# Oscar-W-Chen/gpu-ai-inference-server

Measured on AMD Instinct MI355X. Metric: images/sec, DenseNet-121 fp32, batch 32 per GPU, device-resident inputs, higher is better.
Workload: dtype f32; 1 GPU; DenseNet-121 fp32 batch=32 per GPU, synthetic 3x224x224 inputs (BASELINE configs[1]); synthetic ONNX graph + seeded random weights (reference model file is not in the mount); global_batch=32, per_gpu_batch=32, parallelism=dp1 (independent batch shards)

## Files before the change

gpu-ai-inference-server_amd/csrc/kernels_wino.hip:

```cpp
#include <hip/hip_runtime.h>

#include <algorithm>
#include <cstdlib>
#include <type_traits>

#include "device_util.h"
#include "kernels.h"
#include "launch_util.h"

namespace ie {

__global__ void winograd_weights_kernel(const float* __restrict__ w, float* __restrict__ u, const int Cout, const int Cin) {
    const int idx = blockIdx.x * blockDim.x + threadIdx.x;
    if (idx >= Cout * Cin) return;
    const int co = idx / Cin, ci = idx - co * Cin;
    float g[3][3];
#pragma unroll
    for (int a = 0; a < 3; ++a)
#pragma unroll
        for (int b = 0; b < 3; ++b) g[a][b] = w[((co * 3 + a) * 3 + b) * Cin + ci];
    float t[4][3];
#pragma unroll
    for (int b = 0; b < 3; ++b) {
        t[0][b] = g[0][b];
        t[1][b] = 0.5f * (g[0][b] + g[1][b] + g[2][b]);
        t[2][b] = 0.5f * (g[0][b] - g[1][b] + g[2][b]);
        t[3][b] = g[2][b];
    }
    const int ch8 = ci >> 3, hh = (ci >> 2) & 1, e = ci & 3;
#pragma unroll
    for (int i = 0; i < 4; ++i) {
        const float uu[4] = {t[i][0], 0.5f * (t[i][0] + t[i][1] + t[i][2]), 0.5f * (t[i][0] - t[i][1] + t[i][2]), t[i][2]};
#pragma unroll
        for (int j = 0; j < 4; ++j) {
            const int xi = 4 * i + j;
            u[((int64_t(xi) * (Cin >> 3) + ch8) * 64 + (hh * 32 + co)) * 4 + e] = uu[j];
        }
    }
}

__global__ void winograd_weights_x6_kernel(const float* __restrict__ w, unsigned short* __restrict__ dst, const int Cout, const int Cin) {
    const int idx = blockIdx.x * blockDim.x + threadIdx.x;
    if (idx >= Cout * Cin) return;
    const int co = idx / Cin, ci = idx - co * Cin;
    float g[3][3];
#pragma unroll
    for (int a = 0; a < 3; ++a)
#pragma unroll
        for (int b = 0; b < 3; ++b) g[a][b] = w[((co * 3 + a) * 3 + b) * Cin + ci];
    float t[4][3];
#pragma unroll
    for (int b = 0; b < 3; ++b) {
        t[0][b] = g[0][b];
        t[1][b] = 0.5f * (g[0][b] + g[1][b] + g[2][b]);
        t[2][b] = 0.5f * (g[0][b] - g[1][b] + g[2][b]);
        t[3][b] = g[2][b];
    }
    const int KB = Cin >> 4, kb = ci >> 4, lane = co + 32 * ((ci >> 3) & 1), e = ci & 7;
    const int64_t plane = int64_t(16) * 32 * Cin;
#pragma unroll
    for (int i = 0; i < 4; ++i) {
        const float uu[4] = {t[i][0], 0.5f * (t[i][0] + t[i][1] + t[i][2]), 0.5f * (t[i][0] - t[i][1] + t[i][2]), t[i][2]};
#pragma unroll
        for (int j = 0; j < 4; ++j) {
            const float x = uu[j];
            const unsigned h0 = __builtin_bit_cast(unsigned, x) & 0xffff0000u;
            const float r1 = x - __builtin_bit_cast(float, h0);
            const unsigned h1 = __builtin_bit_cast(unsigned, r1) & 0xffff0000u;
            const unsigned h2 = __builtin_bit_cast(unsigned, r1 - __builtin_bit_cast(float, h1));
            const int64_t off = ((int64_t(4 * i + j) * KB + kb) * 64 + lane) * 8 + e;
            dst[off] = static_cast<unsigned short>(h0 >> 16);
            dst[plane + off] = static_cast<unsigned short>(h1 >> 16);
            dst[2 * plane + off] = static_cast<unsigned short>(h2 >> 16);
        }
    }
}

hipError_t LaunchWinogradWeightsX6(const float* w, void* dst, int Cout, int Cin, hipStream_t stream) {
    if (Cout != 32 || (Cin % 16) || Cin <= 0) return hipErrorInvalidValue;
    const int total = Cout * Cin;
    winograd_weights_x6_kernel<<<dim3((total + 255) / 256), dim3(256), 0, stream>>>(w, static_cast<unsigned short*>(dst), Cout, Cin);
    return hipGetLastError();
}

hipError_t LaunchWinogradWeights(const float* w, float* u, int Cout, int Cin, hipStream_t stream) {
    if (Cout != 32 || (Cin % 16) || Cin <= 0) return hipErrorInvalidValue;
    const int total = Cout * Cin;
    winograd_weights_kernel<<<dim3((total + 255) / 256), dim3(256), 0, stream>>>(w, u, Cout, Cin);
    return hipGetLastError();
}

struct WinoGeom {
    int TR, TC;
    int TH, TW;
    int bry, brx;
};

template <int WAVES, bool X6 = false>
__global__ __launch_bounds__(64 * WAVES) __attribute__((amdgpu_waves_per_eu(2, (WAVES == 8 && !X6) ? 4 : 2))) void conv3x3_wino_kernel(const ConvArgs a, const WinoGeom g) {
    constexpr int NT = 64 * WAVES, CS = 16, LP = CS + 4, MP = 32 + 4, PITW = 1024 / NT;
    constexpr int NJ = 16 / WAVES;
    constexpr unsigned OOB = 0x80000000u;
    extern __shared__ __attribute__((aligned(16))) float smem_wino[];
    const int WR = 2 * g.TR + 2, WC = 2 * g.TC + 2, npx = WR * WC;
    const int win_floats = (npx * LP + 3) & ~3;
    float* const sWin = smem_wino;
    float* const sM = smem_wino;

    const int tid = threadIdx.x, lane = tid & 63, r = lane & 31, hh = lane >> 5;
    const int wave = __builtin_amdgcn_readfirstlane(tid >> 6);
    const int Cin = a.in.c, H = a.in.h, W = a.in.w;
    const int ipitch = int(a.in.sw), opitch = int(a.out.sw);
    int bid = blockIdx.x;
    const int bx = bid % g.brx; bid /= g.brx;
    const int by = bid % g.bry;
    const int b = bid / g.bry;
    const int ty0 = by * g.TR, tx0 = bx * g.TC;
    const int ntr = min(g.TR, g.TH - ty0), ntc = min(g.TC, g.TW - tx0);
    const int y0 = 2 * ty0 - 1, x0 = 2 * tx0 - 1;
    const int ntiles = g.TR * g.TC;

    const __amdgpu_buffer_rsrc_t rs_in = __builtin_amdgcn_make_buffer_rsrc(a.in.p, 0, int(a.in_bytes), kBufferRsrcFlags);
    const __amdgpu_buffer_rsrc_t rs_u = __builtin_amdgcn_make_buffer_rsrc(const_cast<float*>(a.wfrag), 0, 16 * 32 * Cin * 4, kBufferRsrcFlags);

    const int items = npx * 4;
    int woff[PITW];
#pragma unroll
    for (int i = 0; i < PITW; ++i) {
        const int it = tid + i * NT;
        int off = -1;
        if (it < items) {
            const int px = it >> 2, q = it & 3;
            const int wy = px / WC, wx = px - wy * WC;
            const int y = y0 + wy, x = x0 + wx;
            if (unsigned(y) < unsigned(H) && unsigned(x) < unsigned(W)) off = ((b * H + y) * W + x) * ipitch + q * 4;
        }
        woff[i] = off;
    }
    unsigned wvo[PITW];
    float* wlds[2][PITW];
#pragma unroll
    for (int i = 0; i < PITW; ++i) {
        const int it = tid + i * NT;
        wvo[i] = woff[i] >= 0 ? unsigned(woff[i]) * 4u : OOB;
#pragma unroll
        for (int bf = 0; bf < 2; ++bf) wlds[bf][i] = sWin + bf * win_floats + (it >> 2) * LP + (it & 3) * 4;
    }
    f32x4 pvA[PITW], pvB[PITW];
    const int nslices = Cin / CS, nstages = 2 * nslices;
    auto issue_window = [&](f32x4 (&pv)[PITW], int s) {
#pragma unroll
        for (int i = 0; i < PITW; ++i)
            pv[i] = __builtin_bit_cast(f32x4, __builtin_amdgcn_raw_buffer_load_b128(rs_in, wvo[i], (s < nslices ? s : nslices - 1) * CS * 4, 0));
    };
    auto commit_window = [&](const f32x4 (&pv)[PITW], int buf) {
#pragma unroll
        for (int i = 0; i < PITW; ++i)
            if (tid + i * NT < items) *reinterpret_cast<f32x4*>(wlds[buf][i]) = pv[i];
    };
    const int wi = wave / (WAVES / 4), jh = wave % (WAVES / 4);
    const int ra = wi == 0 ? 0 : wi == 2 ? 2 : 1, rb = wi == 2 ? 1 : wi == 3 ? 3 : 2;
    const float sg = wi == 1 ? 1.f : -1.f;
    constexpr int NC = NJ == 4 ? 4 : 3;
    const int ltr = r / g.TC, ltc = r - ltr * g.TC;
    const int col0 = NJ == 4 ? 0 : jh;
    const int dA = ((2 * ltr + ra) * WC + 2 * ltc + col0) * LP + hh * 4, dB = ((2 * ltr + rb) * WC + 2 * ltc + col0) * LP + hh * 4;
    f32x16 acc[NJ];
#pragma unroll
    for (int xl = 0; xl < NJ; ++xl)
#pragma unroll
        for (int e = 0; e < 16; ++e) acc[xl][e] = 0.f;
    if constexpr (X6) {
        static_assert(NJ == 2, "the split variant is written for eight waves");
        const __amdgpu_buffer_rsrc_t rs_ux = __builtin_amdgcn_make_buffer_rsrc(const_cast<void*>(a.w16), 0, 3 * 16 * 32 * Cin * 2, kBufferRsrcFlags);
        const int KB = Cin >> 4;
        const int plane_b = 16 * 32 * Cin * 2;
        u32x4 ux0[NJ][3], ux1[NJ][3];
        auto issue_ux = [&](u32x4 (&ux)[NJ][3], int sl) {
            const int kb = sl < nslices ? sl : nslices - 1;
#pragma unroll
            for (int xl = 0; xl < NJ; ++xl)
#pragma unroll
                for (int p = 0; p < 3; ++p) ux[xl][p] = __builtin_amdgcn_raw_buffer_load_b128(rs_ux, unsigned(lane) * 16u, p * plane_b + ((NJ * wave + xl) * KB + kb) * 1024, 0);
        };
        const float* const qdA[2] = {sWin + dA + hh * 4, sWin + win_floats + dA + hh * 4};
        const float* const qdB[2] = {sWin + dB + hh * 4, sWin + win_floats + dB + hh * 4};
        f32x4 xra[3][2], xrb[3][2];
        auto read_dx = [&](int buf) {
#pragma unroll
            for (int c = 0; c < 3; ++c)
#pragma unroll
                for (int q = 0; q < 2; ++q) {
                    xra[c][q] = *reinterpret_cast<const f32x4*>(qdA[buf] + c * LP + q * 4);
                    xrb[c][q] = *reinterpret_cast<const f32x4*>(qdB[buf] + c * LP + q * 4);
                }
        };
        const float ka0 = jh == 0 ? 1.f : -1.f, ka1 = jh == 0 ? 0.f : 1.f, ka2 = jh == 0 ? -1.f : 0.f;
        const float kb0 = jh == 0 ? 0.f : 1.f, kb1 = jh == 0 ? 1.f : 0.f, kb2 = jh == 0 ? 1.f : -1.f;
        u32x4 axA[NJ][3], axB[NJ][3];
        auto make_ax = [&](u32x4 (&ax)[NJ][3]) {
            f32x4 v[NJ][2];
#pragma unroll
            for (int q = 0; q < 2; ++q) {
                f32x4 m[3];
#pragma unroll
                for (int c = 0; c < 3; ++c) m[c] = xra[c][q] + sg * xrb[c][q];
                v[0][q] = ka0 * m[0] + ka1 * m[1] + ka2 * m[2];
                v[1][q] = kb0 * m[0] + kb1 * m[1] + kb2 * m[2];
            }
#pragma unroll
            for (int xl = 0; xl < NJ; ++xl) {
                unsigned h0[8], h1[8], h2[8];
#pragma unroll
                for (int e = 0; e < 8; ++e) {
                    const float x = v[xl][e >> 2][e & 3];
                    h0[e] = __builtin_bit_cast(unsigned, x);
                    const float r1 = x - __builtin_bit_cast(float, h0[e] & 0xffff0000u);
                    h1[e] = __builtin_bit_cast(unsigned, r1);
                    h2[e] = __builtin_bit_cast(unsigned, r1 - __builtin_bit_cast(float, h1[e] & 0xffff0000u));
                }
#pragma unroll
                for (int d = 0; d < 4; ++d) {
                    ax[xl][0][d] = __builtin_amdgcn_perm(h0[2 * d + 1], h0[2 * d], 0x07060302u);
                    ax[xl][1][d] = __builtin_amdgcn_perm(h1[2 * d + 1], h1[2 * d], 0x07060302u);
                    ax[xl][2][d] = __builtin_amdgcn_perm(h2[2 * d + 1], h2[2 * d], 0x07060302u);
                }
            }
        };
        auto mfmas_x = [&](const u32x4 (&ax)[NJ][3], const u32x4 (&ux)[NJ][3]) {
#pragma unroll
            for (int xl = 0; xl < NJ; ++xl) {
                const bf16x8 a0 = __builtin_bit_cast(bf16x8, ax[xl][0]), a1 = __builtin_bit_cast(bf16x8, ax[xl][1]), a2 = __builtin_bit_cast(bf16x8, ax[xl][2]);
                const bf16x8 b0 = __builtin_bit_cast(bf16x8, ux[xl][0]), b1 = __builtin_bit_cast(bf16x8, ux[xl][1]), b2 = __builtin_bit_cast(bf16x8, ux[xl][2]);
                acc[xl] = __builtin_amdgcn_mfma_f32_32x32x16_bf16(a2, b0, acc[xl], 0, 0, 0);
                acc[xl] = __builtin_amdgcn_mfma_f32_32x32x16_bf16(a1, b1, acc[xl], 0, 0, 0);
                acc[xl] = __builtin_amdgcn_mfma_f32_32x32x16_bf16(a0, b2, acc[xl], 0, 0, 0);
                acc[xl] = __builtin_amdgcn_mfma_f32_32x32x16_bf16(a1, b0, acc[xl], 0, 0, 0);
                acc[xl] = __builtin_amdgcn_mfma_f32_32x32x16_bf16(a0, b1, acc[xl], 0, 0, 0);
                acc[xl] = __builtin_amdgcn_mfma_f32_32x32x16_bf16(a0, b0, acc[xl], 0, 0, 0);
            }
        };
        issue_window(pvA, 0);
        issue_window(pvB, 1);
        issue_ux(ux0, 0);
        commit_window(pvA, 0);
        issue_window(pvA, 2);
        __syncthreads();
        read_dx(0);
        make_ax(axA);
        commit_window(pvB, 1);
        issue_window(pvB, 3);
        __syncthreads();
        auto xslice = [&](auto parity, int sl, u32x4 (&a_cur)[NJ][3], u32x4 (&a_nxt)[NJ][3], u32x4 (&u_cur)[NJ][3], u32x4 (&u_nxt)[NJ][3], f32x4 (&pv_c)[PITW]) {
            constexpr int P = decltype(parity)::value;
            read_dx(P ^ 1);
            issue_ux(u_nxt, sl + 1);
            mfmas_x(a_cur, u_cur);
            make_ax(a_nxt);
#pragma unroll
            for (int i = 0; i < 6 * NJ; ++i) {
                __builtin_amdgcn_sched_group_barrier(0x008, 1, 0);
                __builtin_amdgcn_sched_group_barrier(0x002, 14, 0);
            }
            commit_window(pv_c, P);
            issue_window(pv_c, sl + 4);
            __syncthreads();
        };
        for (int sl = 0; sl < nslices; sl += 2) {
            xslice(std::integral_constant<int, 0>{}, sl, axA, axB, ux0, ux1, pvA);
            xslice(std::integral_constant<int, 1>{}, sl + 1, axB, axA, ux1, ux0, pvB);
        }
    } else {
    const int c8n = Cin >> 3;
    u32x4 ub0[NJ], ub1[NJ];
    auto issue_u = [&](u32x4 (&ub)[NJ], int h) {
#pragma unroll
        for (int xl = 0; xl < NJ; ++xl)
            ub[xl] = __builtin_amdgcn_raw_buffer_load_b128(rs_u, unsigned(lane) * 16u, ((NJ * wave + xl) * c8n + (h < nstages ? h : nstages - 1)) * 1024, 0);
    };
    f32x4 dra[NC], drb[NC];
    const float* const pdA[2] = {sWin + dA, sWin + win_floats + dA};
    const float* const pdB[2] = {sWin + dB, sWin + win_floats + dB};
    auto read_d = [&](int buf, int half) {
#pragma unroll
        for (int c = 0; c < NC; ++c) {
            dra[c] = *reinterpret_cast<const f32x4*>(pdA[buf] + half * 8 + c * LP);
            drb[c] = *reinterpret_cast<const f32x4*>(pdB[buf] + half * 8 + c * LP);
        }
    };
    f32x4 af[NJ];
    auto make_af = [&]() {
        f32x4 m[NC];
#pragma unroll
        for (int c = 0; c < NC; ++c) m[c] = dra[c] + sg * drb[c];
        if constexpr (NJ == 4) {
            af[0] = m[0] - m[2];
            af[1] = m[1] + m[2];
            af[2] = m[2] - m[1];
            af[3] = m[1] - m[3];
        } else if (jh == 0) {
            af[0] = m[0] - m[2];
            af[1] = m[1] + m[2];
        } else {
            af[0] = m[1] - m[0];
            af[1] = m[0] - m[2];
        }
    };
    auto mfmas = [&](const u32x4 (&ub)[NJ]) {
        f32x4 ac[NJ];
#pragma unroll
        for (int xl = 0; xl < NJ; ++xl) ac[xl] = af[xl];
#pragma unroll
        for (int e = 0; e < 4; ++e)
#pragma unroll
            for (int xl = 0; xl < NJ; ++xl)
                acc[xl] = __builtin_amdgcn_mfma_f32_32x32x2f32(ac[xl][e], __builtin_bit_cast(f32x4, ub[xl])[e], acc[xl], 0, 0, 0);
    };

    issue_window(pvA, 0);
    issue_window(pvB, 1);
    issue_u(ub0, 0);
    issue_u(ub1, 1);
    commit_window(pvA, 0);
    issue_window(pvA, 2);
    __syncthreads();
    read_d(0, 0);
    make_af();
    auto slice = [&](auto parity, int s, f32x4 (&pv_next)[PITW]) {
        constexpr int P = decltype(parity)::value;
        read_d(P, 1);
        commit_window(pv_next, P ^ 1);
        mfmas(ub0);
        issue_u(ub0, 2 * s + 2);
        make_af();
        __syncthreads();
        read_d(P ^ 1, 0);
        issue_window(pv_next, s + 3);
        mfmas(ub1);
        issue_u(ub1, 2 * s + 3);
        make_af();
    };
    for (int s = 0; s < nslices; s += 2) {
        slice(std::integral_constant<int, 0>{}, s, pvB);
        slice(std::integral_constant<int, 1>{}, s + 1, pvA);
    }
    }
    __syncthreads();

    const __amdgpu_buffer_rsrc_t rs_out =
        __builtin_amdgcn_make_buffer_rsrc(a.out.p, 0, int((int64_t(a.out.n) * H * W - 1) * opitch * 4 + 32 * 4), kBufferRsrcFlags);
    constexpr int OIT = (32 * 32 + NT - 1) / NT;
    float s0[OIT][4], s1[OIT][4];
#pragma unroll
    for (int half = 0; half < 2; ++half) {
        if (half) __syncthreads();
        if ((wi >> 1) == half) {
#pragma unroll
            for (int xl = 0; xl < NJ; ++xl)
#pragma unroll
                for (int e = 0; e < 16; ++e) sM[((4 * (wi & 1) + NJ * jh + xl) * 32 + (e & 3) + 8 * (e >> 2) + 4 * hh) * MP + r] = acc[xl][e];
        }
        __syncthreads();
#pragma unroll
        for (int k = 0; k < OIT; ++k) {
            const int it = tid + k * NT;
            const int t = it >> 5, c = it & 31;
            if (t < ntiles) {
                const float* const mb = sM + t * MP + c;
#pragma unroll
                for (int j = 0; j < 4; ++j) {
                    const float ma = mb[(0 + j) * 32 * MP], mbv = mb[(4 + j) * 32 * MP];
                    if (half == 0) { s0[k][j] = ma + mbv; s1[k][j] = mbv; }
                    else { s0[k][j] += ma; s1[k][j] = s1[k][j] - ma - mbv; }
                }
            }
        }
    }
#pragma unroll
    for (int k = 0; k < OIT; ++k) {
        const int it = tid + k * NT;
        const int t = it >> 5, c = it & 31;
        if (t >= ntiles) continue;
        const int tr = t / g.TC, tc = t - tr * g.TC;
        float y[2][2];
        y[0][0] = s0[k][0] + s0[k][1] + s0[k][2];
        y[0][1] = s0[k][1] - s0[k][2] - s0[k][3];
        y[1][0] = s1[k][0] + s1[k][1] + s1[k][2];
        y[1][1] = s1[k][1] - s1[k][2] - s1[k][3];
        const float bq = a.bias != nullptr ? a.bias[c] : 0.f;
        const bool tok = tr < ntr && tc < ntc;
        const int oy = 2 * (ty0 + tr), ox = 2 * (tx0 + tc);
#pragma unroll
        for (int dy = 0; dy < 2; ++dy)
#pragma unroll
            for (int dx = 0; dx < 2; ++dx) {
                float v = y[dy][dx] + bq;
                if (a.relu) v = fmaxf(v, 0.f);
                const unsigned off = tok ? unsigned(((b * H + oy + dy) * W + ox + dx) * opitch + c) * 4u : OOB;
                __builtin_amdgcn_raw_buffer_store_b32(__builtin_bit_cast(unsigned, v), rs_out, off, 0, 0);
            }
    }
}

struct WinoTile { int tr, tc; };
constexpr WinoTile kWinoTiles[kNumConvWinoTiles] = {{4, 7}, {2, 14}, {4, 8}, {2, 16}, {4, 7}, {2, 14}, {4, 8}, {2, 16}, {4, 7}, {2, 14}, {4, 8}, {2, 16}};

static size_t wino_lds_bytes(int tr, int tc) {
    const size_t npx = size_t(2 * tr + 2) * (2 * tc + 2);
    const size_t stage = 2 * ((npx * 20 + 3) & ~size_t(3)) * 4, mtx = size_t(8) * 32 * 36 * 4;
    return stage > mtx ? stage : mtx;
}

bool ConvWinoEligible(const ConvArgs& a, int tile) {
    if (tile < 0 || tile >= kNumConvWinoTiles) return false;
    if (a.kh != 3 || a.kw != 3 || a.sh != 1 || a.sw != 1 || a.pt != 1 || a.pl != 1) return false;
    if (a.in.f16 || a.out.f16 || a.in.f8 || a.out.f8 || a.pre_scale != nullptr || a.res.p != nullptr || a.wfrag == nullptr) return false;
    if (a.out.c != 32 || (a.in.c % 32) || a.in.c < 32 || (a.in.h & 1) || (a.in.w & 1)) return false;
    if (a.out.h != a.in.h || a.out.w != a.in.w || a.out.n != a.in.n) return false;
    if (a.in.sc != 1 || a.out.sc != 1 || (a.in.sw & 3) || (a.out.sw & 3)) return false;
    if (a.in.sh != a.in.w * a.in.sw || a.in.sn != a.in.h * a.in.sh || a.out.sh != a.out.w * a.out.sw || a.out.sn != a.out.h * a.out.sh) return false;
    if (!Aligned16(a.in.p) || !Aligned16(a.out.p) || !Aligned16(a.wfrag)) return false;
    if (a.bias && !Aligned16(a.bias)) return false;
    const int64_t M = int64_t(a.in.n) * a.in.h * a.in.w;
    if (M * a.in.sw * 4 >= (int64_t(1) << 31) || M * a.out.sw * 4 >= (int64_t(1) << 31)) return false;
    const WinoTile t = kWinoTiles[tile];
    if ((2 * t.tr + 2) * (2 * t.tc + 2) * 4 > 4 * 256) return false;
    if (tile >= 8 && (a.w16 == nullptr || !Aligned16(a.w16))) return false;
    return t.tr * t.tc <= 32 && wino_lds_bytes(t.tr, t.tc) <= size_t(64) * 1024;
}

hipError_t LaunchConvWino3x3(const ConvArgs& a_in, int tile, hipStream_t stream) {
    if (!ConvWinoEligible(a_in, tile)) return hipErrorInvalidValue;
    ConvArgs a = a_in;
    a.in_bytes = 4 * (int64_t(a.in.n - 1) * a.in.sn + int64_t(a.in.h - 1) * a.in.sh + int64_t(a.in.w - 1) * a.in.sw + a.in.c);
    const WinoTile t = kWinoTiles[tile];
    WinoGeom g;
    g.TR = t.tr; g.TC = t.tc;
    g.TH = a.in.h / 2; g.TW = a.in.w / 2;
    g.bry = (g.TH + g.TR - 1) / g.TR;
    g.brx = (g.TW + g.TC - 1) / g.TC;
    const int64_t blocks = int64_t(a.in.n) * g.bry * g.brx;
    if (blocks >= (int64_t(1) << 31)) return hipErrorInvalidValue;
    if (tile >= 8) conv3x3_wino_kernel<8, true><<<dim3(unsigned(blocks)), dim3(512), wino_lds_bytes(t.tr, t.tc), stream>>>(a, g);
    else if (tile >= 4) conv3x3_wino_kernel<8><<<dim3(unsigned(blocks)), dim3(512), wino_lds_bytes(t.tr, t.tc), stream>>>(a, g);
    else conv3x3_wino_kernel<4><<<dim3(unsigned(blocks)), dim3(256), wino_lds_bytes(t.tr, t.tc), stream>>>(a, g);
    return hipGetLastError();
}

hipError_t InitKernelsWino() {
    hipError_t e = hipFuncSetAttribute(reinterpret_cast<const void*>(&conv3x3_wino_kernel<4>), hipFuncAttributeMaxDynamicSharedMemorySize, 64 * 1024);
    if (e != hipSuccess) return e;
    if ((e = hipFuncSetAttribute(reinterpret_cast<const void*>(&conv3x3_wino_kernel<8>), hipFuncAttributeMaxDynamicSharedMemorySize, 64 * 1024)) != hipSuccess) return e;
    return hipFuncSetAttribute(reinterpret_cast<const void*>(&conv3x3_wino_kernel<8, true>), hipFuncAttributeMaxDynamicSharedMemorySize, 64 * 1024);
}

}
```

Measured before the change: 16590 images/sec.

## Trim index math and instruction overhead in Winograd 3x3 conv kernel

Replaces the integer divisions in window and tile indexing with 24-bit magic-multiply reciprocals, switches to a 3D grid, and fixes the LDS window stride to a constant. It also uses packed fp32 FMA/add for the input transform, specialises the loop on the column-half and ReLU flags at compile time, folds accumulator zeroing into the first MFMA, and simplifies the epilogue addressing with the bias loaded via a buffer load. The goal is fewer VALU and scalar instructions and less register pressure in a hot DenseNet conv kernel. In exchange it adds inline asm with manual s_nop hazards and new eligibility limits, and grows LDS for small tiles.

```diff
diff --git a/gpu-ai-inference-server_amd/csrc/kernels_wino.hip b/gpu-ai-inference-server_amd/csrc/kernels_wino.hip
--- a/gpu-ai-inference-server_amd/csrc/kernels_wino.hip
+++ b/gpu-ai-inference-server_amd/csrc/kernels_wino.hip
@@ -90,10 +90,37 @@
     return hipGetLastError();
 }
 
+namespace {
+
+__device__ __forceinline__ unsigned mul24(unsigned v, unsigned s) {
+    unsigned r;
+    asm("v_mul_u32_u24 %0, %1, %2" : "=v"(r) : "s"(s), "v"(v));
+    return r;
+}
+
+__device__ __forceinline__ f32x2 pk_fma(f32x2 a, f32x2 b, f32x2 c) {
+    f32x2 d;
+    asm("v_pk_fma_f32 %0, %1, %2, %3" : "=v"(d) : "v"(a), "v"(b), "v"(c));
+    return d;
+}
+__device__ __forceinline__ f32x2 pk_add_mfma(f32x2 a, f32x2 b) {
+    f32x2 d;
+    asm("v_pk_add_f32 %0, %1, %2\n\ts_nop 1" : "=v"(d) : "v"(a), "v"(b));
+    return d;
+}
+__device__ __forceinline__ f32x2 pk_sub_mfma(f32x2 a, f32x2 b) {
+    f32x2 d;
+    asm("v_pk_add_f32 %0, %1, %2 neg_lo:[0,1] neg_hi:[0,1]\n\ts_nop 1" : "=v"(d) : "v"(a), "v"(b));
+    return d;
+}
+
+}
+
 struct WinoGeom {
     int TR, TC;
     int TH, TW;
     int bry, brx;
+    unsigned mg20_wc, mg20_tc;
 };
 
 template <int WAVES, bool X6 = false>
@@ -102,8 +129,8 @@
     constexpr int NJ = 16 / WAVES;
     constexpr unsigned OOB = 0x80000000u;
     extern __shared__ __attribute__((aligned(16))) float smem_wino[];
-    const int WR = 2 * g.TR + 2, WC = 2 * g.TC + 2, npx = WR * WC;
-    const int win_floats = (npx * LP + 3) & ~3;
+    const int WR = 2 * g.TR + 2, WC = 2 * g.TC + 2;
+    constexpr int win_floats = 256 * LP;
     float* const sWin = smem_wino;
     float* const sM = smem_wino;
 
@@ -111,10 +138,7 @@
     const int wave = __builtin_amdgcn_readfirstlane(tid >> 6);
     const int Cin = a.in.c, H = a.in.h, W = a.in.w;
     const int ipitch = int(a.in.sw), opitch = int(a.out.sw);
-    int bid = blockIdx.x;
-    const int bx = bid % g.brx; bid /= g.brx;
-    const int by = bid % g.bry;
-    const int b = bid / g.bry;
+    const int bx = blockIdx.x, by = blockIdx.y, b = blockIdx.z;
     const int ty0 = by * g.TR, tx0 = bx * g.TC;
     const int ntr = min(g.TR, g.TH - ty0), ntc = min(g.TC, g.TW - tx0);
     const int y0 = 2 * ty0 - 1, x0 = 2 * tx0 - 1;
@@ -123,28 +147,23 @@
     const __amdgpu_buffer_rsrc_t rs_in = __builtin_amdgcn_make_buffer_rsrc(a.in.p, 0, int(a.in_bytes), kBufferRsrcFlags);
     const __amdgpu_buffer_rsrc_t rs_u = __builtin_amdgcn_make_buffer_rsrc(const_cast<float*>(a.wfrag), 0, 16 * 32 * Cin * 4, kBufferRsrcFlags);
 
-    const int items = npx * 4;
-    int woff[PITW];
+    const unsigned in_corner = unsigned(((b * H + y0) * W + x0) * ipitch) * 4u;
+    const unsigned wy_lo = unsigned(max(0, -y0)), wy_n = unsigned(min(WR, H - y0)) - wy_lo;
+    const unsigned wx_lo = unsigned(max(0, -x0)), wx_n = unsigned(min(WC, W - x0)) - wx_lo;
+    unsigned wvo[PITW];
+    float* wlds[PITW];
 #pragma unroll
     for (int i = 0; i < PITW; ++i) {
-        const int it = tid + i * NT;
-        int off = -1;
-        if (it < items) {
-            const int px = it >> 2, q = it & 3;
-            const int wy = px / WC, wx = px - wy * WC;
-            const int y = y0 + wy, x = x0 + wx;
-            if (unsigned(y) < unsigned(H) && unsigned(x) < unsigned(W)) off = ((b * H + y) * W + x) * ipitch + q * 4;
-        }
-        woff[i] = off;
-    }
-    unsigned wvo[PITW];
-    float* wlds[2][PITW];
-#pragma unroll
-    for (int i = 0; i < PITW; ++i) {
-        const int it = tid + i * NT;
-        wvo[i] = woff[i] >= 0 ? unsigned(woff[i]) * 4u : OOB;
-#pragma unroll
-        for (int bf = 0; bf < 2; ++bf) wlds[bf][i] = sWin + bf * win_floats + (it >> 2) * LP + (it & 3) * 4;
+        const unsigned it = unsigned(tid) + unsigned(i * NT);
+        const unsigned px = it >> 2, q = it & 3u;
+        const unsigned wy = mul24(px, g.mg20_wc) >> 20, wx = px - mul24(wy, unsigned(WC));
+        const bool inside = wy - wy_lo < wy_n && wx - wx_lo < wx_n;
+        wvo[i] = OOB;
+        if (inside) {
+            asm volatile("; ie-mark wino-item i=%0" ::"n"(i));
+            wvo[i] = in_corner + mul24(mul24(wy, unsigned(W)) + wx, unsigned(ipitch) * 4u) + q * 16u;
+        }
+        wlds[i] = reinterpret_cast<float*>(reinterpret_cast<unsigned char*>(smem_wino) + (it + px) * 16u);
     }
     f32x4 pvA[PITW], pvB[PITW];
     const int nslices = Cin / CS, nstages = 2 * nslices;
@@ -155,22 +174,24 @@
     };
     auto commit_window = [&](const f32x4 (&pv)[PITW], int buf) {
 #pragma unroll
-        for (int i = 0; i < PITW; ++i)
-            if (tid + i * NT < items) *reinterpret_cast<f32x4*>(wlds[buf][i]) = pv[i];
+        for (int i = 0; i < PITW; ++i) *reinterpret_cast<f32x4*>(wlds[i] + buf * win_floats) = pv[i];
     };
     const int wi = wave / (WAVES / 4), jh = wave % (WAVES / 4);
     const int ra = wi == 0 ? 0 : wi == 2 ? 2 : 1, rb = wi == 2 ? 1 : wi == 3 ? 3 : 2;
     const float sg = wi == 1 ? 1.f : -1.f;
     constexpr int NC = NJ == 4 ? 4 : 3;
-    const int ltr = r / g.TC, ltc = r - ltr * g.TC;
+    const unsigned ltr = mul24(unsigned(r), g.mg20_tc) >> 20, ltc = unsigned(r) - mul24(ltr, unsigned(g.TC));
     const int col0 = NJ == 4 ? 0 : jh;
-    const int dA = ((2 * ltr + ra) * WC + 2 * ltc + col0) * LP + hh * 4, dB = ((2 * ltr + rb) * WC + 2 * ltc + col0) * LP + hh * 4;
+    const int dlane = int(mul24(mul24(ltr, unsigned(2 * WC)) + 2u * ltc, unsigned(LP))) + hh * 4;
+    int rowA = (ra * WC + col0) * LP, rowB = (rb * WC + col0) * LP;
+    asm("" : "+s"(rowA), "+s"(rowB));
+    const int dA = dlane + rowA, dB = dlane + rowB;
     f32x16 acc[NJ];
-#pragma unroll
-    for (int xl = 0; xl < NJ; ++xl)
-#pragma unroll
-        for (int e = 0; e < 16; ++e) acc[xl][e] = 0.f;
     if constexpr (X6) {
+#pragma unroll
+        for (int xl = 0; xl < NJ; ++xl)
+#pragma unroll
+            for (int e = 0; e < 16; ++e) acc[xl][e] = 0.f;
         static_assert(NJ == 2, "the split variant is written for eight waves");
         const __amdgpu_buffer_rsrc_t rs_ux = __builtin_amdgcn_make_buffer_rsrc(const_cast<void*>(a.w16), 0, 3 * 16 * 32 * Cin * 2, kBufferRsrcFlags);
         const int KB = Cin >> 4;
@@ -183,16 +204,15 @@
 #pragma unroll
                 for (int p = 0; p < 3; ++p) ux[xl][p] = __builtin_amdgcn_raw_buffer_load_b128(rs_ux, unsigned(lane) * 16u, p * plane_b + ((NJ * wave + xl) * KB + kb) * 1024, 0);
         };
-        const float* const qdA[2] = {sWin + dA + hh * 4, sWin + win_floats + dA + hh * 4};
-        const float* const qdB[2] = {sWin + dB + hh * 4, sWin + win_floats + dB + hh * 4};
+        const float* const qdA = sWin + dA + hh * 4, * const qdB = sWin + dB + hh * 4;
         f32x4 xra[3][2], xrb[3][2];
         auto read_dx = [&](int buf) {
 #pragma unroll
             for (int c = 0; c < 3; ++c)
 #pragma unroll
                 for (int q = 0; q < 2; ++q) {
-                    xra[c][q] = *reinterpret_cast<const f32x4*>(qdA[buf] + c * LP + q * 4);
-                    xrb[c][q] = *reinterpret_cast<const f32x4*>(qdB[buf] + c * LP + q * 4);
+                    xra[c][q] = *reinterpret_cast<const f32x4*>(qdA + buf * win_floats + c * LP + q * 4);
+                    xrb[c][q] = *reinterpret_cast<const f32x4*>(qdB + buf * win_floats + c * LP + q * 4);
                 }
         };
         const float ka0 = jh == 0 ? 1.f : -1.f, ka1 = jh == 0 ? 0.f : 1.f, ka2 = jh == 0 ? -1.f : 0.f;
@@ -279,44 +299,58 @@
             ub[xl] = __builtin_amdgcn_raw_buffer_load_b128(rs_u, unsigned(lane) * 16u, ((NJ * wave + xl) * c8n + (h < nstages ? h : nstages - 1)) * 1024, 0);
     };
     f32x4 dra[NC], drb[NC];
-    const float* const pdA[2] = {sWin + dA, sWin + win_floats + dA};
-    const float* const pdB[2] = {sWin + dB, sWin + win_floats + dB};
+    const float* const pdA = sWin + dA, * const pdB = sWin + dB;
     auto read_d = [&](int buf, int half) {
 #pragma unroll
         for (int c = 0; c < NC; ++c) {
-            dra[c] = *reinterpret_cast<const f32x4*>(pdA[buf] + half * 8 + c * LP);
-            drb[c] = *reinterpret_cast<const f32x4*>(pdB[buf] + half * 8 + c * LP);
+            dra[c] = *reinterpret_cast<const f32x4*>(pdA + buf * win_floats + half * 8 + c * LP);
+            drb[c] = *reinterpret_cast<const f32x4*>(pdB + buf * win_floats + half * 8 + c * LP);
         }
     };
     f32x4 af[NJ];
+    const f32x2 sg2 = {sg, sg};
+    auto run = [&](auto jh_) {
+    constexpr int JH = decltype(jh_)::value;
     auto make_af = [&]() {
-        f32x4 m[NC];
-#pragma unroll
-        for (int c = 0; c < NC; ++c) m[c] = dra[c] + sg * drb[c];
-        if constexpr (NJ == 4) {
-            af[0] = m[0] - m[2];
-            af[1] = m[1] + m[2];
-            af[2] = m[2] - m[1];
-            af[3] = m[1] - m[3];
-        } else if (jh == 0) {
-            af[0] = m[0] - m[2];
-            af[1] = m[1] + m[2];
-        } else {
-            af[0] = m[1] - m[0];
-            af[1] = m[0] - m[2];
-        }
-    };
-    auto mfmas = [&](const u32x4 (&ub)[NJ]) {
+        f32x2 v[NJ][2];
+#pragma unroll
+        for (int h = 0; h < 2; ++h) {
+            f32x2 m[NC];
+#pragma unroll
+            for (int c = 0; c < NC; ++c)
+                m[c] = pk_fma(sg2, h ? __builtin_shufflevector(drb[c], drb[c], 2, 3) : __builtin_shufflevector(drb[c], drb[c], 0, 1),
+                              h ? __builtin_shufflevector(dra[c], dra[c], 2, 3) : __builtin_shufflevector(dra[c], dra[c], 0, 1));
+            if constexpr (NJ == 4) {
+                v[0][h] = pk_sub_mfma(m[0], m[2]);
+                v[1][h] = pk_add_mfma(m[1], m[2]);
+                v[2][h] = pk_sub_mfma(m[2], m[1]);
+                v[3][h] = pk_sub_mfma(m[1], m[NC - 1]);
+            } else if constexpr (JH == 0) {
+                v[0][h] = pk_sub_mfma(m[0], m[2]);
+                v[1][h] = pk_add_mfma(m[1], m[2]);
+            } else {
+                v[0][h] = pk_sub_mfma(m[1], m[0]);
+                v[1][h] = pk_sub_mfma(m[0], m[2]);
+            }
+        }
+#pragma unroll
+        for (int xl = 0; xl < NJ; ++xl) af[xl] = __builtin_shufflevector(v[xl][0], v[xl][1], 0, 1, 2, 3);
+    };
+    auto mfmas = [&](const u32x4 (&ub)[NJ], auto first_) {
+        constexpr bool FIRST = decltype(first_)::value;
         f32x4 ac[NJ];
 #pragma unroll
         for (int xl = 0; xl < NJ; ++xl) ac[xl] = af[xl];
 #pragma unroll
         for (int e = 0; e < 4; ++e)
 #pragma unroll
-            for (int xl = 0; xl < NJ; ++xl)
+            for (int xl = 0; xl < NJ; ++xl) {
+                if constexpr (FIRST) { if (e == 0) acc[xl] = f32x16{}; }
                 acc[xl] = __builtin_amdgcn_mfma_f32_32x32x2f32(ac[xl][e], __builtin_bit_cast(f32x4, ub[xl])[e], acc[xl], 0, 0, 0);
-    };
-
+            }
+    };
+
+    asm volatile("; ie-mark wino-prologue jh=%0" ::"n"(JH));
     issue_window(pvA, 0);
     issue_window(pvB, 1);
     issue_u(ub0, 0);
@@ -326,88 +360,116 @@
     __syncthreads();
     read_d(0, 0);
     make_af();
-    auto slice = [&](auto parity, int s, f32x4 (&pv_next)[PITW]) {
+    auto slice = [&](auto parity, int s, f32x4 (&pv_next)[PITW], auto first_) {
         constexpr int P = decltype(parity)::value;
         read_d(P, 1);
         commit_window(pv_next, P ^ 1);
-        mfmas(ub0);
+        mfmas(ub0, first_);
         issue_u(ub0, 2 * s + 2);
         make_af();
         __syncthreads();
         read_d(P ^ 1, 0);
         issue_window(pv_next, s + 3);
-        mfmas(ub1);
+        mfmas(ub1, std::false_type{});
         issue_u(ub1, 2 * s + 3);
         make_af();
     };
-    for (int s = 0; s < nslices; s += 2) {
-        slice(std::integral_constant<int, 0>{}, s, pvB);
-        slice(std::integral_constant<int, 1>{}, s + 1, pvA);
-    }
+    asm volatile("; ie-mark wino-first jh=%0" ::"n"(JH));
+    slice(std::integral_constant<int, 0>{}, 0, pvB, std::true_type{});
+    slice(std::integral_constant<int, 1>{}, 1, pvA, std::false_type{});
+    for (int s = 2; s < nslices; s += 2) {
+        asm volatile("; ie-mark wino-loop jh=%0" ::"n"(JH));
+        slice(std::integral_constant<int, 0>{}, s, pvB, std::false_type{});
+        slice(std::integral_constant<int, 1>{}, s + 1, pvA, std::false_type{});
+    }
+    };
+    if (NJ == 4 || jh == 0) run(std::integral_constant<int, 0>{});
+    else run(std::integral_constant<int, 1>{});
     }
     __syncthreads();
 
-    const __amdgpu_buffer_rsrc_t rs_out =
-        __builtin_amdgcn_make_buffer_rsrc(a.out.p, 0, int((int64_t(a.out.n) * H * W - 1) * opitch * 4 + 32 * 4), kBufferRsrcFlags);
+    const unsigned out_corner = unsigned(((b * H + 2 * ty0) * W + 2 * tx0) * opitch) * 4u;
+    const __amdgpu_buffer_rsrc_t rs_out = __builtin_amdgcn_make_buffer_rsrc(
+        reinterpret_cast<unsigned char*>(a.out.p) + out_corner, 0, int((int64_t(a.out.n) * H * W - 1) * opitch * 4 + 32 * 4 - int64_t(out_corner)), kBufferRsrcFlags);
+    const __amdgpu_buffer_rsrc_t rs_b = __builtin_amdgcn_make_buffer_rsrc(const_cast<float*>(a.bias), 0, a.bias != nullptr ? 32 * 4 : 0, kBufferRsrcFlags);
     constexpr int OIT = (32 * 32 + NT - 1) / NT;
-    float s0[OIT][4], s1[OIT][4];
+    unsigned tid_e = threadIdx.x;
+    asm volatile("" : "+v"(tid_e));
+    const unsigned c = tid_e & 31u, t0 = tid_e >> 5;
+    const float bq = __builtin_bit_cast(float, __builtin_amdgcn_raw_buffer_load_b32(rs_b, c * 4u, 0, 0));
+    const int nlive = (ntiles - wave * 2 + NT / 32 - 1) / (NT / 32);
+    const float* const mrd = sM + (mul24(t0, unsigned(MP)) + c);
+    float* const mwr = sM + (4 * (wi & 1) + NJ * jh) * 32 * MP + (mul24((tid_e >> 3) & 4u, unsigned(MP)) + c);
+    typedef __attribute__((address_space(3))) volatile float lds_vfloat;
+    lds_vfloat* const mwr_v = (lds_vfloat*)mwr;
+    f32x2 s0[OIT][2], s1[OIT][2];
 #pragma unroll
     for (int half = 0; half < 2; ++half) {
         if (half) __syncthreads();
         if ((wi >> 1) == half) {
+            asm volatile("; ie-mark wino-put half=%0" ::"n"(half));
 #pragma unroll
             for (int xl = 0; xl < NJ; ++xl)
 #pragma unroll
-                for (int e = 0; e < 16; ++e) sM[((4 * (wi & 1) + NJ * jh + xl) * 32 + (e & 3) + 8 * (e >> 2) + 4 * hh) * MP + r] = acc[xl][e];
+                for (int e = 0; e < 16; ++e) mwr_v[(xl * 32 + (e & 3) + 8 * (e >> 2)) * MP] = acc[xl][e];
         }
         __syncthreads();
 #pragma unroll
         for (int k = 0; k < OIT; ++k) {
-            const int it = tid + k * NT;
-            const int t = it >> 5, c = it & 31;
-            if (t < ntiles) {
-                const float* const mb = sM + t * MP + c;
-#pragma unroll
-                for (int j = 0; j < 4; ++j) {
-                    const float ma = mb[(0 + j) * 32 * MP], mbv = mb[(4 + j) * 32 * MP];
-                    if (half == 0) { s0[k][j] = ma + mbv; s1[k][j] = mbv; }
-                    else { s0[k][j] += ma; s1[k][j] = s1[k][j] - ma - mbv; }
+            if (k < nlive) {
+                asm volatile("; ie-mark wino-sum half=%0 k=%1" ::"n"(half), "n"(k));
+                const float* const mb = mrd + k * (NT / 32) * MP;
+#pragma unroll
+                for (int jp = 0; jp < 2; ++jp) {
+                    const f32x2 ma = {mb[(0 + 2 * jp) * 32 * MP], mb[(1 + 2 * jp) * 32 * MP]}, mbv = {mb[(4 + 2 * jp) * 32 * MP], mb[(5 + 2 * jp) * 32 * MP]};
+                    if (half == 0) { s0[k][jp] = ma + mbv; s1[k][jp] = mbv; }
+                    else { s0[k][jp] += ma; s1[k][jp] = s1[k][jp] - ma - mbv; }
                 }
             }
         }
     }
-#pragma unroll
-    for (int k = 0; k < OIT; ++k) {
-        const int it = tid + k * NT;
-        const int t = it >> 5, c = it & 31;
-        if (t >= ntiles) continue;
-        const int tr = t / g.TC, tc = t - tr * g.TC;
-        float y[2][2];
-        y[0][0] = s0[k][0] + s0[k][1] + s0[k][2];
-        y[0][1] = s0[k][1] - s0[k][2] - s0[k][3];
-        y[1][0] = s1[k][0] + s1[k][1] + s1[k][2];
-        y[1][1] = s1[k][1] - s1[k][2] - s1[k][3];
-        const float bq = a.bias != nullptr ? a.bias[c] : 0.f;
-        const bool tok = tr < ntr && tc < ntc;
-        const int oy = 2 * (ty0 + tr), ox = 2 * (tx0 + tc);
-#pragma unroll
-        for (int dy = 0; dy < 2; ++dy)
-#pragma unroll
-            for (int dx = 0; dx < 2; ++dx) {
-                float v = y[dy][dx] + bq;
-                if (a.relu) v = fmaxf(v, 0.f);
-                const unsigned off = tok ? unsigned(((b * H + oy + dy) * W + ox + dx) * opitch + c) * 4u : OOB;
-                __builtin_amdgcn_raw_buffer_store_b32(__builtin_bit_cast(unsigned, v), rs_out, off, 0, 0);
-            }
-    }
-}
+    const unsigned dsp[2][2] = {{0u, unsigned(opitch) * 4u}, {unsigned(W * opitch) * 4u, unsigned((W + 1) * opitch) * 4u}};
+    auto finish = [&](auto relu_) {
+        constexpr bool RELU = decltype(relu_)::value;
+#pragma unroll
+        for (int k = 0; k < OIT; ++k) {
+            if (k >= nlive) continue;
+            asm volatile("; ie-mark wino-finish relu=%0 k=%1" ::"n"(int(RELU)), "n"(k));
+            const unsigned t = t0 + unsigned(k * (NT / 32));
+            const unsigned tr = mul24(t, g.mg20_tc) >> 20, tc = t - mul24(tr, unsigned(g.TC));
+            const bool tok = tr < unsigned(ntr) && tc < unsigned(ntc);
+            unsigned off = OOB;
+            if (tok) {
+                asm volatile("; ie-mark wino-offset relu=%0 k=%1" ::"n"(int(RELU)), "n"(k));
+                off = mul24(mul24(tr, unsigned(W)) + tc, unsigned(opitch) * 8u) + c * 4u;
+            }
+            float y[2][2];
+            y[0][0] = s0[k][0][0] + s0[k][0][1] + s0[k][1][0];
+            y[0][1] = s0[k][0][1] - s0[k][1][0] - s0[k][1][1];
+            y[1][0] = s1[k][0][0] + s1[k][0][1] + s1[k][1][0];
+            y[1][1] = s1[k][0][1] - s1[k][1][0] - s1[k][1][1];
+#pragma unroll
+            for (int dy = 0; dy < 2; ++dy)
+#pragma unroll
+                for (int dx = 0; dx < 2; ++dx) {
+                    float v = y[dy][dx] + bq;
+                    if constexpr (RELU) v = fmaxf(v, 0.f);
+                    __builtin_amdgcn_raw_buffer_store_b32(__builtin_bit_cast(unsigned, v), rs_out, off, dsp[dy][dx], 0);
+                }
+        }
+    };
+    if (__builtin_amdgcn_readfirstlane(a.relu ? 1 : 0) != 0) finish(std::true_type{});
+    else finish(std::false_type{});
+}
+
+static unsigned mg20(unsigned d) { return ((1u << 20) + d - 1) / d; }
 
 struct WinoTile { int tr, tc; };
 constexpr WinoTile kWinoTiles[kNumConvWinoTiles] = {{4, 7}, {2, 14}, {4, 8}, {2, 16}, {4, 7}, {2, 14}, {4, 8}, {2, 16}, {4, 7}, {2, 14}, {4, 8}, {2, 16}};
 
 static size_t wino_lds_bytes(int tr, int tc) {
-    const size_t npx = size_t(2 * tr + 2) * (2 * tc + 2);
-    const size_t stage = 2 * ((npx * 20 + 3) & ~size_t(3)) * 4, mtx = size_t(8) * 32 * 36 * 4;
+    (void)tr; (void)tc;
+    const size_t stage = size_t(2) * 256 * 20 * 4, mtx = size_t(8) * 32 * 36 * 4;
     return stage > mtx ? stage : mtx;
 }
 
@@ -423,6 +485,8 @@
     if (a.bias && !Aligned16(a.bias)) return false;
     const int64_t M = int64_t(a.in.n) * a.in.h * a.in.w;
     if (M * a.in.sw * 4 >= (int64_t(1) << 31) || M * a.out.sw * 4 >= (int64_t(1) << 31)) return false;
+    if (a.in.w >= (1 << 19) || a.in.sw >= (int64_t(1) << 21) || a.out.sw >= (int64_t(1) << 21)) return false;
+    if (a.in.n > 65535 || a.in.h / 2 > 65535) return false;
     const WinoTile t = kWinoTiles[tile];
     if ((2 * t.tr + 2) * (2 * t.tc + 2) * 4 > 4 * 256) return false;
     if (tile >= 8 && (a.w16 == nullptr || !Aligned16(a.w16))) return false;
@@ -439,11 +503,12 @@
     g.TH = a.in.h / 2; g.TW = a.in.w / 2;
     g.bry = (g.TH + g.TR - 1) / g.TR;
     g.brx = (g.TW + g.TC - 1) / g.TC;
-    const int64_t blocks = int64_t(a.in.n) * g.bry * g.brx;
-    if (blocks >= (int64_t(1) << 31)) return hipErrorInvalidValue;
-    if (tile >= 8) conv3x3_wino_kernel<8, true><<<dim3(unsigned(blocks)), dim3(512), wino_lds_bytes(t.tr, t.tc), stream>>>(a, g);
-    else if (tile >= 4) conv3x3_wino_kernel<8><<<dim3(unsigned(blocks)), dim3(512), wino_lds_bytes(t.tr, t.tc), stream>>>(a, g);
-    else conv3x3_wino_kernel<4><<<dim3(unsigned(blocks)), dim3(256), wino_lds_bytes(t.tr, t.tc), stream>>>(a, g);
+    g.mg20_wc = mg20(unsigned(2 * g.TC + 2));
+    g.mg20_tc = mg20(unsigned(g.TC));
+    const dim3 grid(unsigned(g.brx), unsigned(g.bry), unsigned(a.in.n));
+    if (tile >= 8) conv3x3_wino_kernel<8, true><<<grid, dim3(512), wino_lds_bytes(t.tr, t.tc), stream>>>(a, g);
+    else if (tile >= 4) conv3x3_wino_kernel<8><<<grid, dim3(512), wino_lds_bytes(t.tr, t.tc), stream>>>(a, g);
+    else conv3x3_wino_kernel<4><<<grid, dim3(256), wino_lds_bytes(t.tr, t.tc), stream>>>(a, g);
     return hipGetLastError();
 }
 
```

Measured after the change: 16740 images/sec, median of 6. Within noise of the previous version (+0.9%).
